# simongoricar/diploma_thesis-distributed_rendering_of_cgi_using_a_render_cluster

Hardware: AMD Instinct MI355X
Metric: job frames/sec at 1/2/4/8 MI355X (04_very-simple); Mrays/s per GPU (higher is better)
Workload: dtype f32

## Files before the change

diploma_thesis-distributed_rendering_of_cgi_using_a_render_cluster_amd/csrc/tiles.hip:

```cpp
#pragma clang fp contract(off)

#include "paths.hpp"

#pragma clang diagnostic push
#pragma clang diagnostic ignored "-Wunused-function"
#define RR_SPLIT_CONSTS FrameConsts
#include "split_kernels.hpp"
#pragma clang diagnostic pop

namespace rr {

namespace {

struct ShadeConsts {
    float3 world;
    float clamp_indirect;
    int max_bounces, max_diffuse, max_glossy, n_lights, n_tris;
};

RR_D void lds_copy(lds_f4w* dst, const float4* __restrict__ src, int n4) {
    const rr_f4v* s = reinterpret_cast<const rr_f4v*>(src);
    for (int i = threadIdx.x; i < n4; i += kBlock) dst[i] = s[i];
}
RR_D uint32_t hull_flags(lds_tri* tris, int n_tris, int i) {
// ... 198 lines not shown
                const int orig = f2i(ca.w);
                if (closer(t, orig, tmin, h)) {
                    h.t = t;
                    h.u = u;
                    h.v = vv;
                    h.idx = i;
                    h.orig = orig;
                }
            }
        }
    }
}
template <bool kCount>
RR_D void camera_hit(const LdsView& v, uint64_t m0, uint64_t m1, float3 d, float tmin, float tmax, Hit& h,
                     TravCount& cnt) {
    set_miss(h, tmax);
    const Shear sh = make_shear_unit(d);
    camera_tris<kCount>(v, m0, m1, sh, sh.kz, tmin, h, cnt);
}

#ifndef RR_TILES_COVERED
#define RR_TILES_COVERED 1
#endif
RR_D void tile_mask(const FrameConsts& fc, const LdsView& v, int n_tris, float x0, float x1, float y0, float y1,
                    uint64_t& m0, uint64_t& m1, int& covered) {
    const float r = fc.filter_reach;
    const float X0 = x0 + 0.5f - r, X1 = x1 + 0.5f + r, Y0 = y0 + 0.5f - r, Y1 = y1 + 0.5f + r;
    const float Wf = (float)fc.W, Hf = (float)fc.H;
    constexpr float kEps = 0x1p-10f;
    uint64_t a = 0, b = 0;
    float best = 0.0f;
    int best_i = -1;
    for (int i = 0; i < n_tris; ++i) {
        const float4 q = lds_ld4(v.cam + kCamF4 * i + kCamRect);
        bool in = !(q.y < X0 || q.x > X1 || q.w < Y0 || q.z > Y1);
        bool cov = true;
        float pl[3] = {0.0f, 0.0f, 0.0f};
        for (int k = 0; k < 3 && in; ++k) {
            const float4 l = lds_ld4(v.cam + kCamF4 * i + kCamRect + 1 + k);
            const float m = l.x * (l.x > 0.0f ? X1 : X0) + l.y * (l.y > 0.0f ? Y1 : Y0) + l.z;
            in = m >= -1.0f;
            cov = cov && l.x * (l.x > 0.0f ? X0 : X1) + l.y * (l.y > 0.0f ? Y0 : Y1) + l.z >= 1.0f;
            pl[k] = l.w;
        }
        if (in) {
            if (i < 64) a |= 1ull << i;
            else b |= 1ull << (i - 64);
            if (cov) {
                const float e = kEps * (fabsf(pl[0]) * Wf + fabsf(pl[1]) * Hf + fabsf(pl[2]));
                const float lo = pl[0] * (pl[0] > 0.0f ? X0 : X1) + pl[1] * (pl[1] > 0.0f ? Y0 : Y1) + pl[2] - e;
                const float hi = pl[0] * (pl[0] > 0.0f ? X1 : X0) + pl[1] * (pl[1] > 0.0f ? Y1 : Y0) + pl[2] + e;
                if (lo > 0.0f && hi * fc.clip_start * (1.0f + kEps) < 1.0f && lo * fc.clip_end > 1.0f + kEps) {
                    if (lo > best) best_i = i;
                    best = fmaxf(best, lo);
                }
            }
        }
    }
    if (best > 0.0f) {
        for (int i = 0; i < n_tris; ++i) {
            const lds_f4w* l = v.cam + kCamF4 * i + kCamRect + 1;
            const float pa = lds_ld4(l).w, pb = lds_ld4(l + 1).w, pc = lds_ld4(l + 2).w;
            const float e = kEps * (fabsf(pa) * Wf + fabsf(pb) * Hf + fabsf(pc));
            const float lo = pa * (pa > 0.0f ? X0 : X1) + pb * (pb > 0.0f ? Y0 : Y1) + pc - e;
            const float hi = pa * (pa > 0.0f ? X1 : X0) + pb * (pb > 0.0f ? Y1 : Y0) + pc + e;
            if (lo > 0.0f && hi < best) {
                if (i < 64) a &= ~(1ull << i);
                else b &= ~(1ull << (i - 64));
            }
        }
    }
    m0 = ((uint64_t)(uint32_t)__builtin_amdgcn_readfirstlane((int)(uint32_t)(a >> 32)) << 32) |
         (uint32_t)__builtin_amdgcn_readfirstlane((int)(uint32_t)a);
    m1 = ((uint64_t)(uint32_t)__builtin_amdgcn_readfirstlane((int)(uint32_t)(b >> 32)) << 32) |
         (uint32_t)__builtin_amdgcn_readfirstlane((int)(uint32_t)b);
    covered = -1;
    if (RR_TILES_COVERED && best_i >= 0 && __popcll(m0) + __popcll(m1) == 1) {
        const int only = m0 ? (int)__builtin_ctzll(m0) : 64 + (int)__builtin_ctzll(m1);
        covered = only == __builtin_amdgcn_readfirstlane(best_i) ? only : -1;
    }
}

constexpr int kTile = 8;
#ifndef RR_TILE_SHARDS
#define RR_TILE_SHARDS 8
#endif
constexpr int kTileShards = RR_TILE_SHARDS;
constexpr int kTileCtrStride = 32;

struct TileOrder {
    int tx, n;
    int bx0, by0, bw, bh;
    RR_D void at(int i, int& x, int& y) const {
        const int nb = bw * bh;
        if (i < nb) {
            y = i / bw;
            x = bx0 + (i - y * bw);
            y += by0;
            return;
        }
        int j = i - nb;
        const int ntop = by0 * tx;
        if (j < ntop) {
            y = j / tx;
            x = j - y * tx;
            return;
        }
        j -= ntop;
        const int rw = tx - bw, nmid = bh * rw;
        if (j < nmid) {
            const int r = j / rw, cx = j - r * rw;
            y = by0 + r;
            x = cx < bx0 ? cx : cx + bw;
            return;
        }
        j -= nmid;
        y = j / tx;
        x = j - y * tx;
        y += by0 + bh;
    }
};

RR_D TileOrder tile_order(const FrameConsts& fc, const ScreenCull& sc) {
    TileOrder to;
    to.tx = (fc.W + kTile - 1) / kTile;
    const int ty = (fc.H + kTile - 1) / kTile;
    to.n = to.tx * ty;
    to.bx0 = to.by0 = 0;
    to.bw = to.tx;
    to.bh = ty;
    if (!sc.on) return to;
    const float m = fc.filter_reach + 1.0f;
    const float x0 = fmaxf(sc.r[0] - m, 0.0f), x1 = fminf(sc.r[1] + m, (float)fc.W - 1.0f);
    const float y0 = fmaxf(sc.r[2] - m, 0.0f), y1 = fminf(sc.r[3] + m, (float)fc.H - 1.0f);
    if (!(x0 <= x1 && y0 <= y1)) {
        to.bw = to.bh = 0;
        return to;
    }
    to.bx0 = (int)x0 / kTile;
    to.by0 = (int)y0 / kTile;
    to.bw = (int)x1 / kTile - to.bx0 + 1;
    to.bh = (int)y1 / kTile - to.by0 + 1;
    return to;
}

struct TileRect {
    int x0, y0, w, h;
};
RR_D TileOrder region_order(const TileOrder& to, const TileRect& rt) {
    TileOrder r;
    r.tx = rt.w;
    r.n = rt.w * rt.h;
    r.bx0 = r.by0 = r.bw = r.bh = 0;
    const int bx0 = max(to.bx0, rt.x0), by0 = max(to.by0, rt.y0);
    const int bx1 = min(to.bx0 + to.bw, rt.x0 + rt.w), by1 = min(to.by0 + to.bh, rt.y0 + rt.h);
    if (to.bw > 0 && to.bh > 0 && bx0 < bx1 && by0 < by1) {
        r.bx0 = bx0 - rt.x0;
        r.by0 = by0 - rt.y0;
        r.bw = bx1 - bx0;
        r.bh = by1 - by0;
    }
    return r;
}

RR_D bool tile_culled(const FrameConsts& fc, const ScreenCull& sc, int tx, int ty) {
    if (!sc.on) return false;
    const float x0 = (float)(tx * kTile) + 0.5f, y0 = (float)(ty * kTile) + 0.5f;
    const float x1 = x0 + (float)(kTile - 1), y1 = y0 + (float)(kTile - 1);
    const float r = fc.filter_reach;
    return x1 + r < sc.r[0] || x0 - r > sc.r[1] || y1 + r < sc.r[2] || y0 - r > sc.r[3];
}
// ... 52 lines not shown
    const bool occ = traverse<true, kCount>(v.nodes, v.tris, n_tris, so, sd, 0.0f, dist, st, hs, cnt);
    if (kCount) {
        __hip_atomic_fetch_add(tt.wctr + 6, cnt.nodes, __ATOMIC_RELAXED, __HIP_MEMORY_SCOPE_WORKGROUP);
        __hip_atomic_fetch_add(tt.wctr + 7, cnt.tris, __ATOMIC_RELAXED, __HIP_MEMORY_SCOPE_WORKGROUP);
    }
    return occ;
}
template <bool kCount>
__device__ __noinline__ Hit ext_trace(LdsView v, int n_tris, float3 o, float3 d, TileTrav tt) {
    wave_add(tt.wctr + 2, wave_count(true));
    TravStack st{tt.lds, tt.spill, tt.stride, 0, tt.drops};
    TravCount cnt;
    Hit h;
    traverse<false, kCount>(v.nodes, v.tris, n_tris, o, d, 0.0f, kFltMax, st, h, cnt);
    if (kCount) {
        __hip_atomic_fetch_add(tt.wctr + 4, cnt.nodes, __ATOMIC_RELAXED, __HIP_MEMORY_SCOPE_WORKGROUP);
        __hip_atomic_fetch_add(tt.wctr + 5, cnt.tris, __ATOMIC_RELAXED, __HIP_MEMORY_SCOPE_WORKGROUP);
    }
    return h;
}
template <bool kCount>
struct InlineShadow {
    static constexpr bool kInline = true;
    LdsView v;
    int n_tris;
    TileTrav tt;
    RR_D bool operator()(float3 so, float3 sd, float dist) const {
        return shadow_trace<kCount>(v, n_tris, so, sd, dist, tt);
    }
};

template <bool kCount>
__device__ __noinline__ float3 tiles_continue(ShadeConsts sc, LdsView v, float3 o, float3 d, float3 T, uint32_t lob,
                                              uint32_t key, float3 L, TileTrav tt) {
    uint32_t nc = 0, ns = 0;
    bool live = true;
    for (int b = 1; b <= sc.max_bounces; ++b) {
        if (!__any(live)) break;
        bool cont = false, shadow = false;
        if (live) {
            ShadeOut so;
            const Hit h = ext_trace<kCount>(v, sc.n_tris, o, d, tt);
            shade(sc, b, v, o, d, T, lob, h, key, L, so, InlineShadow<kCount>{v, sc.n_tris, tt});
            cont = so.cont;
            shadow = so.shadow;
            if (so.cont && so.esc) {
                add_to(L, clamp_contrib(mul3(so.T, sc.world), sc.clamp_indirect));
                live = false;
            } else if (so.cont) {
                o = so.o;
                d = so.d;
                T = so.T;
                lob = so.lob;
            } else {
                live = false;
            }
        }
        nc += wave_count(cont);
        ns += wave_count(shadow);
    }
    wave_add(tt.wctr, nc);
    wave_add(tt.wctr + 1, ns);
    return L;
}

#ifndef RR_TILES_CONT_INPLACE
#define RR_TILES_CONT_INPLACE 1
#endif
template <bool kCount>
struct TileCont {
    static constexpr bool kInline = true;
    ShadeConsts sc;
    LdsView v;
    TileTrav tt;
    uint32_t key;
    RR_D void operator()(float3 o, float3 d, float3 T, uint32_t lob, bool esc, float3& L) const {
        if (esc)
            add_to(L, clamp_contrib(mul3(T, sc.world), sc.clamp_indirect));
        else
            L = tiles_continue<kCount>(sc, v, o, d, T, lob, key, L, tt);
    }
};

}
struct TileSlices {
    int n;
    size_t floats;
    float* slab;
    const int32_t* order;
    uint32_t* cost;
};
namespace {

template <bool kCount, bool kWhole, bool kRegion = false>
RR_D void tiles_body(const FrameConsts& fc, const LdsView& v, uint32_t* __restrict__ tile_ctr, float4* __restrict__ film,
                     const float* __restrict__ srgb, uchar4* __restrict__ out, uint32_t* __restrict__ tot,
                     int32_t* __restrict__ spill, unsigned long long* __restrict__ tc, lds_int* stack,
                     const TileSlices sl, unsigned long long rt_entry, lds_uint* cont_ctr,
                     const TileRect rt = TileRect{0, 0, 0, 0}) {
    const int stride = gridDim.x * kBlock;
    unsigned long long clk0 = 0, rt0 = 0;
    if (kCount) {
        clk0 = __builtin_amdgcn_s_memtime();
        rt0 = __builtin_amdgcn_s_memrealtime();
    }
    const TileTrav tt{stack, spill, stride, tot + drops_slot(fc.max_bounces), cont_ctr + kWctr * (threadIdx.x >> 6), tc};
    TravCount cp;
    uint32_t n_c0 = 0, n_s0 = 0, n_c1 = 0, n_s1 = 0, n_t0 = 0;
    const ScreenCull cull = uniform_cull(screen_cull(fc, v.nodes));
    const TileOrder fto = uniform_order(tile_order(fc, cull));
    const TileOrder to = kRegion ? region_order(fto, rt) : fto;
    const int lane = threadIdx.x & 63;
    const int ng = (fc.spp_total + kFilmGroup - 1) / kFilmGroup;
    const int nb = to.bw * to.bh;
    const int n_slices = kWhole ? 1 : sl.n;
    const int n_sliced = nb * n_slices;
    const int n_units = n_sliced + (to.n - nb);
    const int n_shards = min((int)gridDim.x, kTileShards);
    const int shard = (int)blockIdx.x % n_shards;
    float4 bg = make_float4(0.0f, 0.0f, 0.0f, 0.0f);
    for (int g = 0; g < ng; ++g) {
        float3 P = mk3(0.0f, 0.0f, 0.0f);
        const int s_end = min(fc.spp_total, (g + 1) * kFilmGroup);
        for (int s = g * kFilmGroup; s < s_end; ++s) add_to(P, fc.world);
        bg.x = bg.x + P.x;
        bg.y = bg.y + P.y;
        bg.z = bg.z + P.z;
    }
    bg = make_float4(uniform_f(bg.x), uniform_f(bg.y), uniform_f(bg.z), 0.0f);
    const uchar4 bg_px = __builtin_bit_cast(uchar4, uniform_i(__builtin_bit_cast(int, tonemap(fc, bg, srgb))));
    for (;;) {
        int t, k = 0, nk = 1;
        int u = 0;
        if (lane == 0) u = (int)atomicAdd(tile_ctr + shard * kTileCtrStride, 1u);
        u = __builtin_amdgcn_readlane(u, 0) * n_shards + shard;
        if (u >= n_units) break;
        if (u < n_sliced) {
            const int j = kWhole ? u : u / n_slices;
            k = kWhole ? 0 : u - j * n_slices;
            nk = n_slices;
            t = uniform_i(sl.order[j]);
        } else {
            t = nb + (u - n_sliced);
        }
        const unsigned long long u_start = __builtin_amdgcn_s_memrealtime();
        int tx, ty;
        to.at(t, tx, ty);
        if (kRegion) {
            tx += rt.x0;
            ty += rt.y0;
        }
        const int px = tx * kTile + (lane & (kTile - 1)), py = ty * kTile + (lane >> 3);
        const bool valid = px < fc.W && py < fc.H;
        const int pix = py * fc.W + px;
        float4 acc = make_float4(0.0f, 0.0f, 0.0f, 0.0f);
        if (tile_culled(fc, cull, tx, ty)) {
            if (k != 0) continue;
            if (valid) {
                film[pix] = bg;
                out[pix] = bg_px;
            }
            continue;
        }
        const int s_lo = nk > 1 ? k * kFilmGroup : 0;
        const int s_hi = nk > 1 ? min(fc.spp_total, s_lo + kFilmGroup) : fc.spp_total;
        uint64_t cm0, cm1;
        int cov;
        tile_mask(fc, v, fc.n_tris, (float)(tx * kTile), (float)(tx * kTile + kTile - 1), (float)(ty * kTile),
                  (float)(ty * kTile + kTile - 1), cm0, cm1, cov);
        const uint32_t pk = pixel_key(fc.seed, (uint32_t)pix);
        const int s_run = (cm0 | cm1) != 0 ? s_hi : s_lo;
        float3 P = mk3(0.0f, 0.0f, 0.0f);
        auto group_end = [&](int s) {
            if ((s + 1) % kFilmGroup == 0 || s + 1 == s_hi) {
                acc.x = acc.x + P.x;
                acc.y = acc.y + P.y;
                acc.z = acc.z + P.z;
                P = mk3(0.0f, 0.0f, 0.0f);
            }
        };
        for (int s = s_run; s < s_hi; ++s) {
            add_to(P, fc.world);
            group_end(s);
        }
        bool covered = cov >= 0 && tx * kTile + kTile <= fc.W && ty * kTile + kTile <= fc.H && fc.n_lights <= 1;
        if (covered && cull.on) {
            const float r = fc.filter_reach, cx = (float)(tx * kTile) + 0.5f, cy = (float)(ty * kTile) + 0.5f;
            covered = cx - r >= cull.r[0] && cx + (float)(kTile - 1) + r <= cull.r[1] && cy - r >= cull.r[2] &&
                      cy + (float)(kTile - 1) + r <= cull.r[3];
        }
        int s_gen = s_run;
        if (RR_TILES_COVERED && covered) {
            const float4 nm = lds_ld4(v.nrm + cov), a0 = lds_ld4(v.cam + kCamF4 * cov);
            const bool flip = uniform_i(dot3(xyz(nm), mk3(a0.z, a0.x, a0.y)) > 0.0f ? 1 : 0) != 0;
#if RR_TILES_COVERED == 2
            CoveredHeld held;
            {
                const auto uf3 = [](float3 a) { return mk3(uniform_f(a.x), uniform_f(a.y), uniform_f(a.z)); };
                const int word = uniform_i(f2i(nm.w));
                held.mid = word & ((1 << kHullShift) - 1);
                held.esc = ((((uint32_t)word >> kHullShift) >> (flip ? 1 : 0)) & 1u) != 0u;
                held.N = uf3(flip ? mk3(-nm.x, -nm.y, -nm.z) : xyz(nm));
                const Mat m = view_mat(v, held.mid);
                held.m.base = uf3(m.base);
                held.m.roughness = uniform_f(m.roughness);
                held.m.emission = uf3(m.emission);
                held.m.model = uniform_i(m.model);
                held.m.alpha = uniform_f(m.alpha);
                held.m.a2 = uniform_f(m.a2);
                held.m.kd0 = uniform_f(m.kd0);
                held.m.spec_on = uniform_i(m.spec_on);
                held.m.cspec0 = uf3(m.cspec0);
                held.m.metallic = held.m.specular = held.m.ior = 0.0f;
                const lds_f4w* fr = v.onb + kOnbF4 * cov + (flip ? 2 : 0);
                const float4 tb = lds_ld4(fr), bb = lds_ld4(fr + 1);
                held.tb = uf3(xyz(tb));
                held.bb = uf3(mk3(tb.w, bb.x, bb.y));
                for (int k = 0; k < 11; ++k) held.lt[k] = fc.n_lights > 0 ? uniform_f(v.lights[k]) : 0.0f;
            }
#else
            const CoveredInLoop held;
#endif
            for (int s = s_lo; s < s_hi; ++s) {
                const uint32_t key = sample_key(pk, (uint32_t)s);
                float3 o, d, L = mk3(0.0f, 0.0f, 0.0f);
                float tmin, tmax;
                camera_ray_xy(fc, v.filter, px, py, key, o, d, tmin, tmax);
                n_t0 += 64u;
                const Shear sh = make_shear_unit(d);
                if (kCount) ++cp.tris;
                const lds_f4w* q = v.cam + kCamF4 * cov + 3 * sh.kz;
                const float4 ca = lds_ld4(q), cb = lds_ld4(q + 1), cc = lds_ld4(q + 2);
                Hit h;
                set_miss(h, tmax);
                float t = tmax, u, vv;
                bool hit = woop_core(sh, xyz(ca), xyz(cb), xyz(cc), t, u, vv);
                hit = hit && closer(t, f2i(ca.w), tmin, h);
                h.t = hit ? t : tmax;
                ShadeOut so;
                const ShadeConsts sc{fc.world, fc.clamp_indirect, fc.max_bounces, fc.max_diffuse, fc.max_glossy,
                                     fc.n_lights, fc.n_tris};
                if constexpr ((RR_TILES_CONT_INPLACE & (kWhole ? 1 : 2)) != 0) {
                    shade_covered(fc, 0, v, cov, flip, hit, o, d, mk3(1.0f, 1.0f, 1.0f), 0u, h, key, L, so,
                                  InlineShadow<kCount>{v, fc.n_tris, tt}, TileCont<kCount>{sc, v, tt, key}, held);
                } else {
                    shade_covered(fc, 0, v, cov, flip, hit, o, d, mk3(1.0f, 1.0f, 1.0f), 0u, h, key, L, so,
                                  InlineShadow<kCount>{v, fc.n_tris, tt}, EmitCont{}, held);
                    if (so.cont) TileCont<kCount>{sc, v, tt, key}(so.o, so.d, so.T, so.lob, so.esc, L);
                }
                n_c0 += wave_count(so.cont);
                n_s0 += wave_count(so.shadow);
                add_to(P, L);
// ... 43 lines not shown
            out[pix] = tonemap(fc, acc, srgb);
        }
        if (lane == 0) {
            const unsigned long long u_end = __builtin_amdgcn_s_memrealtime();
            atomicAdd(&sl.cost[ty * fto.tx + tx], (uint32_t)(u_end - u_start));
            if ((kCount || RR_TILES_LOG_ALWAYS) && u < kUnitLog) {
                tc[kTravWords + 2 * u] = u_start;
                tc[kTravWords + 2 * u + 1] = u_end;
            }
        }
    }
    uint32_t* const tail = tot + camera_traced_slot(fc.max_bounces);
    n_c1 = tt.wctr[0];
    n_s1 = tt.wctr[1];
    flush_rays(tot, n_c0, n_s0, n_c1, n_s1, tail, n_t0, tt.wctr[2], tt.wctr[3]);
    if (kCount && lane == 0) {
        atomicAdd(&tc[2], (unsigned long long)tt.wctr[4]);
        atomicAdd(&tc[3], (unsigned long long)tt.wctr[5]);
        atomicAdd(&tc[4], (unsigned long long)tt.wctr[6]);
        atomicAdd(&tc[5], (unsigned long long)tt.wctr[7]);
    }
    if (kCount) {
        flush_counts(tc, 0, cp.nodes, cp.tris);
        const unsigned long long clk1 = __builtin_amdgcn_s_memtime(), rt1 = __builtin_amdgcn_s_memrealtime();
        if ((threadIdx.x & 63) == 0) {
            atomicAdd(&tc[6], clk1 - clk0);
            atomicAdd(&tc[7], rt1 - rt0);
            atomicAdd(&tc[8], 1ull);
            atomicAdd(&tc[9], rt1 - rt_entry);
            atomicMax(&tc[10], ~rt_entry);
            atomicMax(&tc[11], rt1);
            atomicMax(&tc[12], rt_entry);
            atomicMax(&tc[13], ~rt1);
        }
    }
}

#ifndef RR_TILES_WAVES
#define RR_TILES_WAVES 4
#endif
#ifndef RR_TILES_WAVES_WHOLE
#define RR_TILES_WAVES_WHOLE 5
#endif
template <bool kCount, bool kWhole>
__global__ __launch_bounds__(kBlock, kWhole ? RR_TILES_WAVES_WHOLE : RR_TILES_WAVES) void k_tiles(FrameConsts fc,
                                                                                                 SceneArgs sa,
                                                                  uint32_t* __restrict__ tile_ctr,
                                                                  float4* __restrict__ film,
                                                                  const float* __restrict__ srgb,
                                                                  uchar4* __restrict__ out, uint32_t* __restrict__ tot,
                                                                  int32_t* __restrict__ spill,
                                                                  unsigned long long* __restrict__ tc,
                                                                  TileSlices sl) {
    const unsigned long long rt_entry = kCount ? __builtin_amdgcn_s_memrealtime() : 0ull;
    __shared__ int lds_stack[kLdsStack * kBlock];
    __shared__ uint32_t cont_ctr[kWctr * kWavesPerBlock];
    extern __shared__ float4 dyn4[];
    lds_int* stack = lds_slot(lds_stack);
    if (threadIdx.x < kWctr * kWavesPerBlock) cont_ctr[threadIdx.x] = 0u;
    int used;
    const LdsView v = stage_scene<true>((lds_f4w*)dyn4, sa, true, used, &fc);
    tiles_body<kCount, kWhole>(fc, v, tile_ctr, film, srgb, out, tot, spill, tc, stack, sl, rt_entry,
                               (lds_uint*)cont_ctr);
}

constexpr int kOrderBuckets = 128;
constexpr int kOrderThreads = 1024;
RR_D int cost_bucket(uint32_t c) {
    if (c < 4u) return (int)c;
    const int e = 31 - __builtin_clz(c);
    return min(kOrderBuckets - 1, 4 * e + (int)((c >> (e - 2)) & 3u));
}
template <bool kRegion>
RR_D void tile_order_body(const FrameConsts& fc, const BvhNode* __restrict__ nodes, uint32_t* __restrict__ cost,
                          int32_t* __restrict__ order, uint32_t* __restrict__ tile_ctr,
                          uint32_t* __restrict__ ray_ctr, int n_ray_ctr, const TileRect rt) {
    __shared__ uint32_t cnt[kOrderBuckets];
    const int tid = threadIdx.x;
    const ScreenCull cull = screen_cull(fc, nodes);
    const TileOrder fto = tile_order(fc, cull);
    const TileOrder to = kRegion ? region_order(fto, rt) : fto;
    const int nb = to.bw * to.bh;
    for (int i = tid; i < kOrderBuckets; i += kOrderThreads) cnt[i] = 0u;
    for (int i = tid; i < kTileShards * kTileCtrStride; i += kOrderThreads) tile_ctr[i] = 0u;
    for (int i = tid; i < n_ray_ctr; i += kOrderThreads) ray_ctr[i] = 0u;
    __syncthreads();
    for (int t = tid; t < nb; t += kOrderThreads) {
        int x, y;
        to.at(t, x, y);
        if (kRegion) {
            x += rt.x0;
            y += rt.y0;
        }
        atomicAdd(&cnt[cost_bucket(cost[y * fto.tx + x])], 1u);
    }
    __syncthreads();
    if (tid == 0) {
        uint32_t run = 0;
        for (int b = kOrderBuckets - 1; b >= 0; --b) {
            const uint32_t c = cnt[b];
            cnt[b] = run;
            run += c;
        }
    }
    __syncthreads();
    for (int t = tid; t < nb; t += kOrderThreads) {
        int x, y;
        to.at(t, x, y);
        if (kRegion) {
            x += rt.x0;
            y += rt.y0;
        }
        order[atomicAdd(&cnt[cost_bucket(cost[y * fto.tx + x])], 1u)] = t;
    }
    __syncthreads();
    for (int i = tid; i < fto.n; i += kOrderThreads) cost[i] = 0u;
}
__global__ __launch_bounds__(kOrderThreads) void k_tile_order(FrameConsts fc, const BvhNode* __restrict__ nodes,
                                                              uint32_t* __restrict__ cost, int32_t* __restrict__ order,
                                                              uint32_t* __restrict__ tile_ctr,
                                                              uint32_t* __restrict__ ray_ctr, int n_ray_ctr) {
    tile_order_body<false>(fc, nodes, cost, order, tile_ctr, ray_ctr, n_ray_ctr, TileRect{0, 0, 0, 0});
}

template <bool kRegion>
RR_D void tiles_fold_body(const FrameConsts& fc, const BvhNode* __restrict__ nodes, const TileSlices& sl,
                          float4* __restrict__ film, const float* __restrict__ srgb, uchar4* __restrict__ out,
                          const TileRect rt) {
    const ScreenCull cull = screen_cull(fc, nodes);
    const TileOrder to = kRegion ? region_order(tile_order(fc, cull), rt) : tile_order(fc, cull);
    const int nb = to.bw * to.bh;
    const int lane = threadIdx.x & 63;
    const int wave = blockIdx.x * kWavesPerBlock + (threadIdx.x >> 6);
    for (int t = wave; t < nb; t += gridDim.x * kWavesPerBlock) {
        int tx, ty;
        to.at(t, tx, ty);
        if (kRegion) {
            tx += rt.x0;
            ty += rt.y0;
        }
        if (tile_culled(fc, cull, tx, ty)) continue;
        const int px = tx * kTile + (lane & (kTile - 1)), py = ty * kTile + (lane >> 3);
        if (px >= fc.W || py >= fc.H) continue;
        const float* slab = sl.slab + (size_t)t * sl.floats;
        float4 acc = make_float4(0.0f, 0.0f, 0.0f, 0.0f);
        for (int g = 0; g < sl.n; ++g, slab += 192) {
            acc.x = acc.x + slab[lane];
            acc.y = acc.y + slab[64 + lane];
            acc.z = acc.z + slab[128 + lane];
        }
        const int pix = py * fc.W + px;
        film[pix] = acc;
        out[pix] = tonemap(fc, acc, srgb);
    }
}
__global__ __launch_bounds__(kBlock) void k_tiles_fold(FrameConsts fc, const BvhNode* __restrict__ nodes,
                                                       TileSlices sl, float4* __restrict__ film,
                                                       const float* __restrict__ srgb, uchar4* __restrict__ out) {
    tiles_fold_body<false>(fc, nodes, sl, film, srgb, out, TileRect{0, 0, 0, 0});
}

template <bool kCount, bool kWhole>
__global__ __launch_bounds__(kBlock, kWhole ? RR_TILES_WAVES_WHOLE : RR_TILES_WAVES) void k_tiles_region(
    FrameConsts fc, SceneArgs sa, uint32_t* __restrict__ tile_ctr, float4* __restrict__ film,
    const float* __restrict__ srgb, uchar4* __restrict__ out, uint32_t* __restrict__ tot, int32_t* __restrict__ spill,
    unsigned long long* __restrict__ tc, TileSlices sl, TileRect rt) {
    const unsigned long long rt_entry = kCount ? __builtin_amdgcn_s_memrealtime() : 0ull;
    __shared__ int lds_stack[kLdsStack * kBlock];
    __shared__ uint32_t cont_ctr[kWctr * kWavesPerBlock];
    extern __shared__ float4 dyn4[];
    lds_int* stack = lds_slot(lds_stack);
    if (threadIdx.x < kWctr * kWavesPerBlock) cont_ctr[threadIdx.x] = 0u;
    int used;
    const LdsView v = stage_scene<true>((lds_f4w*)dyn4, sa, true, used, &fc);
    tiles_body<kCount, kWhole, true>(fc, v, tile_ctr, film, srgb, out, tot, spill, tc, stack, sl, rt_entry,
                                     (lds_uint*)cont_ctr, rt);
}
__global__ __launch_bounds__(kOrderThreads) void k_tile_order_region(FrameConsts fc, const BvhNode* __restrict__ nodes,
                                                                     uint32_t* __restrict__ cost,
                                                                     int32_t* __restrict__ order,
                                                                     uint32_t* __restrict__ tile_ctr,
                                                                     uint32_t* __restrict__ ray_ctr, int n_ray_ctr,
                                                                     TileRect rt) {
    tile_order_body<true>(fc, nodes, cost, order, tile_ctr, ray_ctr, n_ray_ctr, rt);
}
__global__ __launch_bounds__(kBlock) void k_tiles_fold_region(FrameConsts fc, const BvhNode* __restrict__ nodes,
                                                              TileSlices sl, float4* __restrict__ film,
                                                              const float* __restrict__ srgb, uchar4* __restrict__ out,
                                                              TileRect rt) {
    tiles_fold_body<true>(fc, nodes, sl, film, srgb, out, rt);
}

int film_groups(int spp) { return (spp + kFilmGroup - 1) / kFilmGroup; }
size_t tile_slab_bytes(int spp, long tiles) {
    const int ng = film_groups(spp);
    return ng > 1 ? (size_t)192 * sizeof(float) * ng * (size_t)tiles : 0;
}
constexpr size_t kTileSlabMax = (size_t)16 << 30;
size_t scene_lds_bytes(const FrameConsts& fc, bool shading) {
    const int n_nodes = std::max(fc.n_tris - 1, 1);
    size_t f4 = 4 * (size_t)n_nodes + kTriF4 * (size_t)fc.n_tris;
    if (shading)
        f4 += (3 + kMatDF4 + kMatLutStride / 4) * (size_t)fc.n_mats + 3 * (size_t)fc.n_lights + kFilterN / 4 +
              (size_t)(1 + kOnbF4) * fc.n_tris;
    return 16 * f4;
}
}

constexpr size_t kTilesStaticLds = sizeof(int) * (size_t)(kLdsStack * kBlock + kWctr * kWavesPerBlock);
size_t tiles_dyn_lds_bytes(const FrameConsts& fc) {
    return scene_lds_bytes(fc, true) + 16 * (size_t)kCamF4 * (size_t)fc.n_tris;
}
constexpr int kTilesMinBlocks = 3;
constexpr size_t kCuLds = 160 * 1024;
bool scene_in_lds(int n_tris, int n_mats, int n_lights) {
    FrameConsts fc{};
    fc.n_tris = n_tris;
    fc.n_mats = n_mats;
    fc.n_lights = n_lights;
    return n_tris > 0 && n_tris <= 128 &&
           kTilesMinBlocks * (kTilesStaticLds + tiles_dyn_lds_bytes(fc)) <= kCuLds;
}

bool frame_uses_tiles(const FrameConsts& base, bool force_wavefront) {
    const long n_tiles = (long)((base.W + 7) / 8) * ((base.H + 7) / 8);
    return scene_in_lds(base.n_tris, base.n_mats, base.n_lights) && !force_wavefront &&
           tile_slab_bytes(base.spp_total, n_tiles) <= kTileSlabMax;
}

long long tiles_pixels_run(int W, int H, bool region_on, const RegionRect& r) {
    if (!region_on) return (long long)W * H;
    const int x0 = r.x0 / kTile * kTile, y0 = r.y0 / kTile * kTile;
    const int x1 = std::min(W, (r.x1 + kTile - 1) / kTile * kTile), y1 = std::min(H, (r.y1 + kTile - 1) / kTile * kTile);
    return (long long)(x1 - x0) * (y1 - y0);
}

namespace {
TileRect region_tiles(const RegionRect& r) {
    if (r.empty()) return TileRect{0, 0, 0, 0};
    const int x0 = r.x0 / kTile, y0 = r.y0 / kTile;
    return TileRect{x0, y0, (r.x1 + kTile - 1) / kTile - x0, (r.y1 + kTile - 1) / kTile - y0};
}
struct TileGrid {
    decltype(&k_tiles<false, false>) kx;
    decltype(&k_tiles_region<false, false>) kxr = nullptr;
    size_t dyn;
    int grid;
    TileGrid(const FrameConsts& fc, bool count, bool whole, bool region) {
        dyn = tiles_dyn_lds_bytes(fc);
        kx = count ? (whole ? k_tiles<true, true> : k_tiles<true, false>)
                   : (whole ? k_tiles<false, true> : k_tiles<false, false>);
        if (region) {
            kxr = count ? (whole ? k_tiles_region<true, true> : k_tiles_region<true, false>)
                        : (whole ? k_tiles_region<false, true> : k_tiles_region<false, false>);
            grid = grid_for(kxr, dyn);
        } else {
            grid = grid_for(kx, dyn);
        }
    }
};
}

void render_tiles_device(const DevMesh& m, DevBuild& s, DevPaths& p, DevFrame& f, const FrameConsts& base, int n_chunks,
                         FrameOpts o, hipStream_t st) {
    const int npix = base.npix;
    const TileGrid G(base, o.count_traversal, o.tile_whole, o.region_on);
    if (p.grid_blocks == 0) p.grid_blocks = device_cu_count() * kMaxBlocksPerCu;
    f.ensure_spill(p.grid_blocks);
    f.film.ensure((size_t)npix);
    f.rgba8.ensure((size_t)npix * 4);
    const int cpc = counters_per_chunk(base.max_bounces);
    const long tiles = (long)((base.W + 7) / 8) * ((base.H + 7) / 8);
    const size_t n_ctr = (size_t)cpc * n_chunks;
    f.counters.ensure(n_ctr);
    unsigned long long* tc = nullptr;
    if (o.count_traversal || RR_TILES_LOG_ALWAYS) {
        f.trav_counts.ensure(kTravWords + 2 * kUnitLog);
        RR_HIP(hipMemsetAsync(f.trav_counts.ptr, 0, (kTravWords + 2 * kUnitLog) * sizeof(unsigned long long), st));
        tc = f.trav_counts.ptr;
        f.unit_logged = true;
    }
    const SceneArgs sa{s.nodes.ptr, s.qnodes.ptr, s.tris.ptr, f.materials.ptr, f.lights.ptr, p.filter_table.ptr,
                       f.mat_lut.ptr, std::max(m.n_tris - 1, 1), m.n_tris, base.n_mats, base.n_lights, s.nq};
    FrameConsts fc = base;
    fc.first_sample = 0;
    fc.spp_chunk = base.spp_total;
    uint32_t* tot = reinterpret_cast<uint32_t*>(f.counters.ptr);
    if (f.tile_cost.cap < 2 * (size_t)tiles) {
        f.tile_cost.ensure(2 * (size_t)tiles);
        RR_HIP(hipMemsetAsync(f.tile_cost.ptr, 0, sizeof(uint32_t) * tiles, st));
    }
    if (o.count_traversal)
        RR_HIP(hipMemsetAsync(f.tile_cost.ptr + tiles, 0, sizeof(uint32_t) * tiles, st));
    f.tile_order.ensure((size_t)tiles);
    TileSlices sl{o.tile_whole ? 1 : film_groups(base.spp_total), (size_t)192 * film_groups(base.spp_total), nullptr,
                  f.tile_order.ptr, f.tile_cost.ptr};
    f.tile_slices = sl.n;
    const TileRect rt = region_tiles(o.region);
    const long tiles_run = o.region_on ? (long)rt.w * rt.h : tiles;
    if (sl.n > 1) {
        f.tile_slab.ensure(sl.floats * (size_t)tiles_run);
        sl.slab = f.tile_slab.ptr;
    }
    const int g = clamp_grid(tiles_run * 64, G.grid);
    f.prof.begin(st, RR_K_TILES);
    f.tile_ctrs.ensure((size_t)kTileShards * kTileCtrStride);
    const int g_fold = (int)std::min<long>((tiles_run + kWavesPerBlock - 1) / kWavesPerBlock, 2048);
    if (o.region_on) {
        k_tile_order_region<<<1, kOrderThreads, 0, st>>>(fc, s.nodes.ptr, f.tile_cost.ptr, f.tile_order.ptr,
                                                         f.tile_ctrs.ptr, reinterpret_cast<uint32_t*>(f.counters.ptr),
                                                         (int)n_ctr, rt);
        G.kxr<<<g, kBlock, G.dyn, st>>>(fc, sa, f.tile_ctrs.ptr, f.film.ptr, p.srgb_lut.ptr,
                                        reinterpret_cast<uchar4*>(f.rgba8.ptr), tot, f.spill.ptr, tc, sl, rt);
        if (sl.n > 1)
            k_tiles_fold_region<<<g_fold, kBlock, 0, st>>>(fc, s.nodes.ptr, sl, f.film.ptr, p.srgb_lut.ptr,
                                                           reinterpret_cast<uchar4*>(f.rgba8.ptr), rt);
        f.prof.end(st);
        RR_HIP(hipGetLastError());
        return;
    }
    k_tile_order<<<1, kOrderThreads, 0, st>>>(fc, s.nodes.ptr, f.tile_cost.ptr, f.tile_order.ptr, f.tile_ctrs.ptr,
                                              reinterpret_cast<uint32_t*>(f.counters.ptr), (int)n_ctr);
    G.kx<<<g, kBlock, G.dyn, st>>>(fc, sa, f.tile_ctrs.ptr, f.film.ptr, p.srgb_lut.ptr,
                                           reinterpret_cast<uchar4*>(f.rgba8.ptr), tot, f.spill.ptr, tc, sl);
    if (sl.n > 1)
        k_tiles_fold<<<g_fold, kBlock, 0, st>>>(
            fc, s.nodes.ptr, sl, f.film.ptr, p.srgb_lut.ptr, reinterpret_cast<uchar4*>(f.rgba8.ptr));
    f.prof.end(st);
    RR_HIP(hipGetLastError());
}

}
```

diploma_thesis-distributed_rendering_of_cgi_using_a_render_cluster_amd/native.py:

```python
from __future__ import annotations

import ctypes
import os
from dataclasses import dataclass

import numpy as np

_HERE = os.path.dirname(os.path.abspath(__file__))
LIB_PATH = os.path.join(_HERE, "lib", "librr.so")
SHIM_PATH = os.path.join(_HERE, "lib", "rr-blender-shim")

RR_OK, RR_ENOENT, RR_EIO, RR_ENOMEM, RR_ENODEV, RR_EINVAL, RR_ENOTSUP = 0, -2, -5, -12, -19, -22, -95
RR_EBUSY = -16
RR_MAX_FRAMES_IN_FLIGHT = 3
RR_MAX_FRAME_OUTPUTS = 4
RR_VIEW_SCENE, RR_VIEW_STANDARD, RR_VIEW_RAW, RR_VIEW_FILMIC = -1, 0, 1, 2
RR_VIEW_FILMIC_LOG, RR_VIEW_FALSE_COLOR = 3, 4
LOOKS = ["None", "Very High Contrast", "High Contrast", "Medium High Contrast", "Medium Contrast",
         "Medium Low Contrast", "Low Contrast", "Very Low Contrast"]
RR_ABI_VERSION = 8
QWIDTH = 6
RR_CAM_FLOATS, RR_LIGHT_FLOATS, RR_MAT_FLOATS, RR_RENDER_INTS, RR_RENDER_FLOATS = 16, 12, 12, 10, 4


# ... 611 lines not shown
        v = RR_DITHER_SCENE if intensity == "scene" else float(intensity)
        _check(lib().rr_set_dither(self.handle, ctypes.c_float(v)), self.handle)

    def set_png_compression(self, percent="legacy"):
        _check(lib().rr_set_png_compression(self.handle, png_compression_value(percent)), self.handle)

    def view_device(self, rgba: np.ndarray, view_transform: int = 0, exposure_scale: float = 1.0) -> np.ndarray:
        rgba = np.ascontiguousarray(rgba, dtype=np.float32)
        h, w = rgba.shape[:2]
        out = np.zeros((h, w, 4), np.uint8)
        _check(lib().rr_debug_view_device(self.handle, _ptr(rgba, ctypes.c_float), w, h, int(view_transform),
                                          ctypes.c_float(exposure_scale), _ptr(out, ctypes.c_uint8)), self.handle)
        return out

    def encode_device(self, fmt: str, image: np.ndarray, depth: int = 0, color_mode=0, view_transform: int = 0,
                      exposure_scale: float = 1.0, quality: int = 90) -> bytes:
        if fmt == "HDR" and (image.dtype == np.uint8 or int(depth) not in (0, 32)):
            raise RRError(RR_EINVAL, "HDR takes a float image at depth 0 or 32")
        is_float = image.dtype != np.uint8
        image = np.ascontiguousarray(image, dtype=np.float32 if is_float else np.uint8)
        h, w = image.shape[:2]
        args = (self.handle, fmt.encode(), int(depth), color_mode_value(color_mode),
                image.ctypes.data_as(ctypes.c_void_p), 1 if is_float else 0, w, h, int(view_transform),
                ctypes.c_float(exposure_scale), int(quality))
        n = ctypes.c_uint64()
        _check(lib().rr_debug_encode_device(*args, None, 0, ctypes.byref(n)), self.handle)
        out = np.zeros(n.value, np.uint8)
        _check(lib().rr_debug_encode_device(*args, _ptr(out, ctypes.c_uint8), out.size, ctypes.byref(n)), self.handle)
        if n.value > out.size:
            raise RRError(RR_EINVAL, f"device file of {n.value} bytes exceeds the {out.size}-byte buffer")
        return out[:n.value].tobytes()

    def exr32_device(self, rgba: np.ndarray) -> bytes:
        rgba = np.ascontiguousarray(rgba, dtype=np.float32)
        h, w = rgba.shape[:2]
        out = np.zeros(16 * w * h + 16 * ((h + 15) // 16) + 1024, np.uint8)
        n = ctypes.c_uint64()
        _check(lib().rr_debug_exr32_device(self.handle, _ptr(rgba, ctypes.c_float), w, h,
                                           _ptr(out, ctypes.c_uint8), out.size, ctypes.byref(n)), self.handle)
        if n.value > out.size:
            raise RRError(RR_EINVAL, f"device EXR of {n.value} bytes exceeds the {out.size}-byte buffer")
        return out[:n.value].tobytes()

    def bsdf_sample(self, mat12, n, wo, u):
        f32 = lambda a: np.ascontiguousarray(a, dtype=np.float32)
        m, n, wo, u = f32(mat12), f32(n), f32(wo), f32(u).reshape(-1, 3)
        k = u.shape[0]
        wi, f = np.zeros((k, 3), np.float32), np.zeros((k, 3), np.float32)
        pdf, ok = np.zeros(k, np.float32), np.zeros(k, np.int32)
        _check(lib().rr_debug_bsdf_sample(self.handle, _ptr(m, ctypes.c_float), _ptr(n, ctypes.c_float),
                                          _ptr(wo, ctypes.c_float), k, _ptr(u, ctypes.c_float),
                                          _ptr(wi, ctypes.c_float), _ptr(f, ctypes.c_float),
                                          _ptr(pdf, ctypes.c_float), _ptr(ok, ctypes.c_int32)), self.handle)
        return wi, f, pdf, ok

    def fastmath_check(self, lo: int = 0, n: int = 1 << 32):
        out = (ctypes.c_uint64 * 5)()
        _check(lib().rr_debug_fastmath_check(self.handle, int(lo), int(n), out), self.handle)
        return tuple(int(v) for v in out)

    def tile_costs(self, capacity: int = 1 << 20, units: int = 1 << 16, raw: bool = False):
        costs = np.zeros(capacity, np.uint32)
        order = np.zeros(capacity, np.int32)
        log = np.zeros((max(units, 1), 2), np.uint64)
        n = ctypes.c_int32(0)
        _check(lib().rr_debug_tile_costs(self.handle, capacity, _ptr(costs, ctypes.c_uint32),
                                         _ptr(order, ctypes.c_int32), ctypes.byref(n),
                                         _ptr(log, ctypes.c_uint64), units), self.handle)
        m = min(int(n.value), capacity)
        return (costs if raw else costs[:m]), order[:m], log[:units]

    def trace(self, scene: Scene, frame: int, rays: np.ndarray, width: int = 0):
        rays = np.ascontiguousarray(rays, dtype=np.float32).reshape(-1, 8)
        n = rays.shape[0]
        hits = np.zeros((max(n, 1), 4), np.float32)
        prims = np.zeros(max(n, 1), np.int32)
        occ = np.zeros(max(n, 1), np.uint8)
        _check(lib().rr_debug_trace(self.handle, scene.handle, int(frame), int(width), n, _ptr(rays, ctypes.c_float),
                                    _ptr(hits, ctypes.c_float), _ptr(prims, ctypes.c_int32),
                                    _ptr(occ, ctypes.c_uint8)), self.handle)
        return hits[:n], prims[:n], occ[:n]


def srgb16_table() -> np.ndarray:
    n = ctypes.c_int32()
    _check(lib().rr_debug_srgb16_table(None, 0, ctypes.byref(n)))
    t = np.zeros(n.value, np.float32)
    _check(lib().rr_debug_srgb16_table(_ptr(t, ctypes.c_float), t.size, ctypes.byref(n)))
    return t


def display_gamma(values: np.ndarray, gamma: float) -> np.ndarray:
    v = np.ascontiguousarray(values, dtype=np.float32)
    out = np.zeros_like(v)
    _check(lib().rr_debug_display_gamma(_ptr(v.reshape(-1), ctypes.c_float), v.size, ctypes.c_float(gamma),
                                        _ptr(out.reshape(-1), ctypes.c_float)))
    return out


def sin_fixed(values: np.ndarray) -> np.ndarray:
    v = np.ascontiguousarray(values, dtype=np.float32)
    out = np.zeros_like(v)
    _check(lib().rr_debug_sin_fixed(_ptr(v.reshape(-1), ctypes.c_float), v.size, _ptr(out.reshape(-1), ctypes.c_float)))
    return out


def dither_noise(width: int, height: int) -> np.ndarray:
    out = np.zeros((int(height), int(width)), np.float32)
    _check(lib().rr_debug_dither_noise(int(width), int(height), _ptr(out.reshape(-1), ctypes.c_float)))
    return out


def encode_image(rgba: np.ndarray, out_path_no_ext: str, fmt: str, quality: int = 90) -> int:
    rgba = np.ascontiguousarray(rgba, dtype=np.uint8)
    h, w = rgba.shape[:2]
    nbytes = ctypes.c_uint64()
    _check(lib().rr_encode_image(_ptr(rgba, ctypes.c_uint8), w, h, out_path_no_ext.encode(), fmt.encode(),
                                 int(quality), ctypes.byref(nbytes)))
    return nbytes.value


def last_host_warning() -> str:
    return lib().rr_last_warning(None).decode("utf-8", "replace")


def encode_image_mode(rgba: np.ndarray, out_path_no_ext: str, fmt: str, quality: int = 90, color_mode=0) -> int:
    rgba = np.ascontiguousarray(rgba, dtype=np.uint8)
    h, w = rgba.shape[:2]
    nbytes = ctypes.c_uint64()
    _check(lib().rr_encode_image_mode(_ptr(rgba, ctypes.c_uint8), w, h, out_path_no_ext.encode(), fmt.encode(),
                                      int(quality), color_mode_value(color_mode), ctypes.byref(nbytes)))
    return nbytes.value


def encode_image_png(rgba: np.ndarray, out_path_no_ext: str, color_mode=0, compression="legacy") -> int:
    rgba = np.ascontiguousarray(rgba, dtype=np.uint8)
    h, w = rgba.shape[:2]
    nbytes = ctypes.c_uint64()
    _check(lib().rr_encode_image_png(_ptr(rgba, ctypes.c_uint8), w, h, out_path_no_ext.encode(),
                                     color_mode_value(color_mode), png_compression_value(compression),
                                     ctypes.byref(nbytes)))
    return nbytes.value


def hdr_host(rgba: np.ndarray, color_mode=0) -> bytes:
    rgba = np.ascontiguousarray(rgba, dtype=np.float32)
    h, w = rgba.shape[:2]
    args = (_ptr(rgba, ctypes.c_float), w, h, color_mode_value(color_mode))
    n = ctypes.c_uint64()
    _check(lib().rr_debug_hdr_host(*args, None, 0, ctypes.byref(n)))
    out = np.zeros(n.value, np.uint8)
    _check(lib().rr_debug_hdr_host(*args, _ptr(out, ctypes.c_uint8), out.size, ctypes.byref(n)))
    return out[:n.value].tobytes()


def png_filters(raw: np.ndarray, bpp: int) -> np.ndarray:
    raw = np.ascontiguousarray(raw, dtype=np.uint8)
    rows, row_bytes = raw.shape
    out = np.zeros(rows, np.uint8)
    _check(lib().rr_debug_png_filters(_ptr(raw.reshape(-1), ctypes.c_uint8), row_bytes, rows, int(bpp),
                                      _ptr(out, ctypes.c_uint8)))
    return out


def film_reduce(rgba: np.ndarray, reduce: int, ctx: "RenderContext | None" = None) -> np.ndarray:
    rgba = np.ascontiguousarray(rgba, dtype=np.float32)
# ... 23 lines not shown
```

Measured before the change: 1331.

## Split lean covered tiles into a dedicated low-register kernel ahead of main tiles

Adds a specialised kernel that renders only the tiles fully covered by a single triangle whose hull flag says no shadow or continuation work is needed. It uses trivial shadow and continuation functors and a higher waves-per-EU occupancy target. The main tile kernel gets a variant that skips these tiles, and it uses a second set of tile counters plus an extra cost segment. The goal is to keep the simple tiles from paying the register and occupancy cost of the full path-tracing kernel. In exchange it adds a second launch, and it runs tile_mask and unit_lean twice for each tile.

Result: slower. 1250 (-6.1%).

```diff
diff --git a/diploma_thesis-distributed_rendering_of_cgi_using_a_render_cluster_amd/csrc/tiles.hip b/diploma_thesis-distributed_rendering_of_cgi_using_a_render_cluster_amd/csrc/tiles.hip
--- a/diploma_thesis-distributed_rendering_of_cgi_using_a_render_cluster_amd/csrc/tiles.hip
+++ b/diploma_thesis-distributed_rendering_of_cgi_using_a_render_cluster_amd/csrc/tiles.hip
@@ -304,11 +304,15 @@
 }
 
 constexpr int kTile = 8;
+#ifndef RR_TILES_LEAN
+#define RR_TILES_LEAN 1
+#endif
 #ifndef RR_TILE_SHARDS
 #define RR_TILE_SHARDS 8
 #endif
 constexpr int kTileShards = RR_TILE_SHARDS;
 constexpr int kTileCtrStride = 32;
+constexpr int kTileCtrSets = RR_TILES_LEAN ? 2 : 1;
 
 struct TileOrder {
     int tx, n;
@@ -527,6 +531,19 @@
     }
 };
 
+struct LeanShadow {
+    static constexpr bool kInline = true;
+    RR_D bool operator()(float3, float3, float) const { return false; }
+};
+struct LeanCont {
+    static constexpr bool kInline = true;
+    float3 world;
+    float clamp_indirect;
+    RR_D void operator()(float3, float3, float3 T, uint32_t, bool, float3& L) const {
+        add_to(L, clamp_contrib(mul3(T, world), clamp_indirect));
+    }
+};
+
 }
 struct TileSlices {
     int n;
@@ -537,7 +554,27 @@
 };
 namespace {
 
-template <bool kCount, bool kWhole, bool kRegion = false>
+RR_D bool tile_covered(const FrameConsts& fc, const ScreenCull& cull, int tx, int ty, int cov) {
+    bool covered = cov >= 0 && tx * kTile + kTile <= fc.W && ty * kTile + kTile <= fc.H && fc.n_lights <= 1;
+    if (covered && cull.on) {
+        const float r = fc.filter_reach, cx = (float)(tx * kTile) + 0.5f, cy = (float)(ty * kTile) + 0.5f;
+        covered = cx - r >= cull.r[0] && cx + (float)(kTile - 1) + r <= cull.r[1] && cy - r >= cull.r[2] &&
+                  cy + (float)(kTile - 1) + r <= cull.r[3];
+    }
+    return covered;
+}
+RR_D bool covered_flip(const float4 nm, const float4 a0) {
+    return uniform_i(dot3(xyz(nm), mk3(a0.z, a0.x, a0.y)) > 0.0f ? 1 : 0) != 0;
+}
+RR_D bool unit_lean(const FrameConsts& fc, const LdsView& v, const ScreenCull& cull, int tx, int ty, int cov) {
+    if (!tile_covered(fc, cull, tx, ty, cov)) return false;
+    const float4 nm = lds_ld4(v.nrm + cov), a0 = lds_ld4(v.cam + kCamF4 * cov);
+    const bool flip = covered_flip(nm, a0);
+    const uint32_t hull = (uint32_t)uniform_i(f2i(nm.w)) >> kHullShift;
+    return ((hull >> (flip ? 1 : 0)) & 1u) != 0u;
+}
+
+template <bool kCount, bool kWhole, bool kRegion = false, bool kSkipLean = false>
 RR_D void tiles_body(const FrameConsts& fc, const LdsView& v, uint32_t* __restrict__ tile_ctr, float4* __restrict__ film,
                      const float* __restrict__ srgb, uchar4* __restrict__ out, uint32_t* __restrict__ tot,
                      int32_t* __restrict__ spill, unsigned long long* __restrict__ tc, lds_int* stack,
@@ -613,6 +650,9 @@
         int cov;
         tile_mask(fc, v, fc.n_tris, (float)(tx * kTile), (float)(tx * kTile + kTile - 1), (float)(ty * kTile),
                   (float)(ty * kTile + kTile - 1), cm0, cm1, cov);
+        if constexpr (kSkipLean) {
+            if (unit_lean(fc, v, cull, tx, ty, cov)) continue;
+        }
         const uint32_t pk = pixel_key(fc.seed, (uint32_t)pix);
         const int s_run = (cm0 | cm1) != 0 ? s_hi : s_lo;
         float3 P = mk3(0.0f, 0.0f, 0.0f);
@@ -822,7 +862,7 @@
     const TileOrder to = kRegion ? region_order(fto, rt) : fto;
     const int nb = to.bw * to.bh;
     for (int i = tid; i < kOrderBuckets; i += kOrderThreads) cnt[i] = 0u;
-    for (int i = tid; i < kTileShards * kTileCtrStride; i += kOrderThreads) tile_ctr[i] = 0u;
+    for (int i = tid; i < kTileCtrSets * kTileShards * kTileCtrStride; i += kOrderThreads) tile_ctr[i] = 0u;
     for (int i = tid; i < n_ray_ctr; i += kOrderThreads) ray_ctr[i] = 0u;
     __syncthreads();
     for (int t = tid; t < nb; t += kOrderThreads) {
@@ -855,6 +895,8 @@
     }
     __syncthreads();
     for (int i = tid; i < fto.n; i += kOrderThreads) cost[i] = 0u;
+    if (RR_TILES_LEAN)
+        for (int i = tid; i < fto.n; i += kOrderThreads) cost[2 * fto.n + i] = 0u;
 }
 __global__ __launch_bounds__(kOrderThreads) void k_tile_order(FrameConsts fc, const BvhNode* __restrict__ nodes,
                                                               uint32_t* __restrict__ cost, int32_t* __restrict__ order,
@@ -931,6 +973,106 @@
     tiles_fold_body<true>(fc, nodes, sl, film, srgb, out, rt);
 }
 
+#if RR_TILES_LEAN
+__global__ __launch_bounds__(kBlock, RR_TILES_WAVES_WHOLE) void k_tiles_skip_lean(
+    FrameConsts fc, SceneArgs sa, uint32_t* __restrict__ tile_ctr, float4* __restrict__ film,
+    const float* __restrict__ srgb, uchar4* __restrict__ out, uint32_t* __restrict__ tot, int32_t* __restrict__ spill,
+    unsigned long long* __restrict__ tc, TileSlices sl) {
+    __shared__ int lds_stack[kLdsStack * kBlock];
+    __shared__ uint32_t cont_ctr[kWctr * kWavesPerBlock];
+    extern __shared__ float4 dyn4[];
+    lds_int* stack = lds_slot(lds_stack);
+    if (threadIdx.x < kWctr * kWavesPerBlock) cont_ctr[threadIdx.x] = 0u;
+    int used;
+    const LdsView v = stage_scene<true>((lds_f4w*)dyn4, sa, true, used, &fc);
+    tiles_body<false, true, false, true>(fc, v, tile_ctr, film, srgb, out, tot, spill, tc, stack, sl, 0ull,
+                                         (lds_uint*)cont_ctr);
+}
+
+#ifndef RR_TILES_LEAN_WAVES
+#define RR_TILES_LEAN_WAVES 6
+#endif
+template <int kWaves>
+__global__ __launch_bounds__(kBlock, kWaves) void k_tiles_lean(FrameConsts fc, SceneArgs sa,
+                                                               uint32_t* __restrict__ tile_ctr,
+                                                               float4* __restrict__ film,
+                                                               const float* __restrict__ srgb,
+                                                               uchar4* __restrict__ out, uint32_t* __restrict__ tot,
+                                                               TileSlices sl) {
+    extern __shared__ float4 dyn4[];
+    int used;
+    const LdsView v = stage_scene<true>((lds_f4w*)dyn4, sa, true, used, &fc);
+    uint32_t n_c0 = 0, n_s0 = 0, n_t0 = 0;
+    const ScreenCull cull = uniform_cull(screen_cull(fc, v.nodes));
+    const TileOrder to = uniform_order(tile_order(fc, cull));
+    const int lane = threadIdx.x & 63;
+    const int nb = to.bw * to.bh;
+    const int n_shards = min((int)gridDim.x, kTileShards);
+    const int shard = (int)blockIdx.x % n_shards;
+    const int s_hi = fc.spp_total;
+    for (;;) {
+        int u = 0;
+        if (lane == 0) u = (int)atomicAdd(tile_ctr + shard * kTileCtrStride, 1u);
+        u = __builtin_amdgcn_readlane(u, 0) * n_shards + shard;
+        if (u >= nb) break;
+        const int t = uniform_i(sl.order[u]);
+        const unsigned long long u_start = __builtin_amdgcn_s_memrealtime();
+        int tx, ty;
+        to.at(t, tx, ty);
+        if (tile_culled(fc, cull, tx, ty)) continue;
+        uint64_t cm0, cm1;
+        int cov;
+        tile_mask(fc, v, fc.n_tris, (float)(tx * kTile), (float)(tx * kTile + kTile - 1), (float)(ty * kTile),
+                  (float)(ty * kTile + kTile - 1), cm0, cm1, cov);
+        if (!unit_lean(fc, v, cull, tx, ty, cov)) continue;
+        const int px = tx * kTile + (lane & (kTile - 1)), py = ty * kTile + (lane >> 3);
+        const int pix = py * fc.W + px;
+        const uint32_t pk = pixel_key(fc.seed, (uint32_t)pix);
+        float4 acc = make_float4(0.0f, 0.0f, 0.0f, 0.0f);
+        float3 P = mk3(0.0f, 0.0f, 0.0f);
+        const float4 nm = lds_ld4(v.nrm + cov), a0 = lds_ld4(v.cam + kCamF4 * cov);
+        const bool flip = covered_flip(nm, a0);
+        const CoveredInLoop held;
+        for (int s = 0; s < s_hi; ++s) {
+            const uint32_t key = sample_key(pk, (uint32_t)s);
+            float3 o, d, L = mk3(0.0f, 0.0f, 0.0f);
+            float tmin, tmax;
+            camera_ray_xy(fc, v.filter, px, py, key, o, d, tmin, tmax);
+            n_t0 += 64u;
+            const Shear sh = make_shear_unit(d);
+            const lds_f4w* q = v.cam + kCamF4 * cov + 3 * sh.kz;
+            const float4 ca = lds_ld4(q), cb = lds_ld4(q + 1), cc = lds_ld4(q + 2);
+            Hit h;
+            set_miss(h, tmax);
+            float th = tmax, bu, bv;
+            bool hit = woop_core(sh, xyz(ca), xyz(cb), xyz(cc), th, bu, bv);
+            hit = hit && closer(th, f2i(ca.w), tmin, h);
+            h.t = hit ? th : tmax;
+            ShadeOut so;
+            shade_covered(fc, 0, v, cov, flip, hit, o, d, mk3(1.0f, 1.0f, 1.0f), 0u, h, key, L, so, LeanShadow{},
+                          LeanCont{fc.world, fc.clamp_indirect}, held);
+            n_c0 += wave_count(so.cont);
+            n_s0 += wave_count(so.shadow);
+            add_to(P, L);
+            if ((s + 1) % kFilmGroup == 0 || s + 1 == s_hi) {
+                acc.x = acc.x + P.x;
+                acc.y = acc.y + P.y;
+                acc.z = acc.z + P.z;
+                P = mk3(0.0f, 0.0f, 0.0f);
+            }
+        }
+        film[pix] = acc;
+        out[pix] = tonemap(fc, acc, srgb);
+        if (lane == 0) {
+            const unsigned long long u_end = __builtin_amdgcn_s_memrealtime();
+            atomicAdd(&sl.cost[ty * to.tx + tx], (uint32_t)(u_end - u_start));
+            sl.cost[2 * to.n + ty * to.tx + tx] = 1u;
+        }
+    }
+    flush_rays(tot, n_c0, n_s0, 0u, 0u, tot + camera_traced_slot(fc.max_bounces), n_t0, 0u, 0u);
+}
+#endif
+
 int film_groups(int spp) { return (spp + kFilmGroup - 1) / kFilmGroup; }
 size_t tile_slab_bytes(int spp, long tiles) {
     const int ng = film_groups(spp);
@@ -986,10 +1128,19 @@
     decltype(&k_tiles_region<false, false>) kxr = nullptr;
     size_t dyn;
     int grid;
+    bool lean = false;
+    int lean_grid = 0;
     TileGrid(const FrameConsts& fc, bool count, bool whole, bool region) {
         dyn = tiles_dyn_lds_bytes(fc);
         kx = count ? (whole ? k_tiles<true, true> : k_tiles<true, false>)
                    : (whole ? k_tiles<false, true> : k_tiles<false, false>);
+#if RR_TILES_LEAN
+        lean = whole && !region && !count;
+        if (lean) {
+            kx = k_tiles_skip_lean;
+            lean_grid = grid_for(k_tiles_lean<RR_TILES_LEAN_WAVES>, dyn);
+        }
+#endif
         if (region) {
             kxr = count ? (whole ? k_tiles_region<true, true> : k_tiles_region<true, false>)
                         : (whole ? k_tiles_region<false, true> : k_tiles_region<false, false>);
@@ -1026,9 +1177,9 @@
     fc.first_sample = 0;
     fc.spp_chunk = base.spp_total;
     uint32_t* tot = reinterpret_cast<uint32_t*>(f.counters.ptr);
-    if (f.tile_cost.cap < 2 * (size_t)tiles) {
-        f.tile_cost.ensure(2 * (size_t)tiles);
-        RR_HIP(hipMemsetAsync(f.tile_cost.ptr, 0, sizeof(uint32_t) * tiles, st));
+    if (f.tile_cost.cap < 3 * (size_t)tiles) {
+        f.tile_cost.ensure(3 * (size_t)tiles);
+        RR_HIP(hipMemsetAsync(f.tile_cost.ptr, 0, sizeof(uint32_t) * 3 * tiles, st));
     }
     if (o.count_traversal)
         RR_HIP(hipMemsetAsync(f.tile_cost.ptr + tiles, 0, sizeof(uint32_t) * tiles, st));
@@ -1044,7 +1195,7 @@
     }
     const int g = clamp_grid(tiles_run * 64, G.grid);
     f.prof.begin(st, RR_K_TILES);
-    f.tile_ctrs.ensure((size_t)kTileShards * kTileCtrStride);
+    f.tile_ctrs.ensure((size_t)kTileCtrSets * kTileShards * kTileCtrStride);
     const int g_fold = (int)std::min<long>((tiles_run + kWavesPerBlock - 1) / kWavesPerBlock, 2048);
     if (o.region_on) {
         k_tile_order_region<<<1, kOrderThreads, 0, st>>>(fc, s.nodes.ptr, f.tile_cost.ptr, f.tile_order.ptr,
@@ -1061,6 +1212,12 @@
     }
     k_tile_order<<<1, kOrderThreads, 0, st>>>(fc, s.nodes.ptr, f.tile_cost.ptr, f.tile_order.ptr, f.tile_ctrs.ptr,
                                               reinterpret_cast<uint32_t*>(f.counters.ptr), (int)n_ctr);
+#if RR_TILES_LEAN
+    if (G.lean)
+        k_tiles_lean<RR_TILES_LEAN_WAVES><<<clamp_grid(tiles_run * 64, G.lean_grid), kBlock, G.dyn, st>>>(
+            fc, sa, f.tile_ctrs.ptr + kTileShards * kTileCtrStride, f.film.ptr, p.srgb_lut.ptr,
+            reinterpret_cast<uchar4*>(f.rgba8.ptr), tot, sl);
+#endif
     G.kx<<<g, kBlock, G.dyn, st>>>(fc, sa, f.tile_ctrs.ptr, f.film.ptr, p.srgb_lut.ptr,
                                            reinterpret_cast<uchar4*>(f.rgba8.ptr), tot, f.spill.ptr, tc, sl);
     if (sl.n > 1)
diff --git a/diploma_thesis-distributed_rendering_of_cgi_using_a_render_cluster_amd/native.py b/diploma_thesis-distributed_rendering_of_cgi_using_a_render_cluster_amd/native.py
--- a/diploma_thesis-distributed_rendering_of_cgi_using_a_render_cluster_amd/native.py
+++ b/diploma_thesis-distributed_rendering_of_cgi_using_a_render_cluster_amd/native.py
@@ -717,6 +717,18 @@
         return hits[:n], prims[:n], occ[:n]
 
 
+TILE_COST_SEGMENTS = 3
+
+
+def tile_cost_segments(raw: np.ndarray, width: int, height: int):
+    tx, ty = (int(width) + 7) // 8, (int(height) + 7) // 8
+    n = tx * ty
+    raw = np.asarray(raw)
+    if n <= 0 or raw.ndim != 1 or raw.shape[0] < TILE_COST_SEGMENTS * n:
+        raise ValueError(f"{raw.shape} words do not hold {TILE_COST_SEGMENTS} segments of {tx} x {ty} tiles")
+    return tuple(raw[k * n:(k + 1) * n].reshape(ty, tx) for k in range(TILE_COST_SEGMENTS))
+
+
 def srgb16_table() -> np.ndarray:
     n = ctypes.c_int32()
     _check(lib().rr_debug_srgb16_table(None, 0, ctypes.byref(n)))
```
